# tonyjohnvan/ACE-Step-1.5

Measured on AMD Instinct MI355X. Metric: seconds/song (240 s audio, 27 DiT steps), lower is better.
Workload: dtype bf16

## Files before the change

ace-step-1.5_amd/csrc/gemm.hip:

```cpp
#include <hip/hip_ext.h>

#include "kernels.h"
#include "headpost.h"

namespace acehip {
namespace {

constexpr int BK = 64;
constexpr int GROUP_M = 8;

#ifdef GEMM_STAMPS
constexpr int STAMP_WG = 16384;
__device__ unsigned long long g_gemm_stamps[STAMP_WG * 2 * 8];
__device__ __forceinline__ void stamp(int slot, int i, unsigned long long v) {
    if (slot < STAMP_WG * 2) {
        asm volatile("" : "+v"(v));
        g_gemm_stamps[slot * 8 + i] = v;
    }
}
#define GSTAMP_AT(slot, i)                                                                       \
    do {                                                                                         \
        if ((threadIdx.x & 255) == 0 && threadIdx.x < 512) stamp((slot) * 2 + (threadIdx.x >> 8), i, __builtin_amdgcn_s_memtime()); \
    } while (0)
#define GSTAMP_REAL_AT(slot, i)                                                                  \
// ... 465 lines not shown
        asm volatile("s_getreg_b32 %0, hwreg(HW_REG_XCC_ID)" : "=s"(xcc));
        if ((threadIdx.x & 255) == 0) {
            stamp(slot * 2 + (threadIdx.x >> 8), 6, ((unsigned long long)wg << 32) | xcc);
            stamp(slot * 2 + (threadIdx.x >> 8), 7, blockIdx.x);
        }
    }
#endif
}

template <int BM>
struct PPSrcPtr {
    static constexpr int NA = BM / 64, NB = 4;
    const bf16_t *pa[NA], *pb[NB];
    __device__ __forceinline__ void set(const GemmArgs &a, int m0, int n0, int wave, int lane) {
#pragma unroll
        for (int i = 0; i < NA; ++i) {
            const int r = (wave + 8 * i) * 8 + (lane >> 3);
            const int c = (lane & 7) ^ ((r >> 1) & 7);
            pa[i] = a.A + (int64_t)min(m0 + r, a.M - 1) * a.lda + c * 8;
        }
#pragma unroll
        for (int i = 0; i < NB; ++i) {
            const int r = (wave + 8 * i) * 8 + (lane >> 3);
            const int c = (lane & 7) ^ (((BM + r) >> 1) & 7);
            pb[i] = a.W + (int64_t)(n0 + r) * a.ldw + c * 8;
        }
    }
    __device__ __forceinline__ void dmaA(int i, int k0, char *dst) const { glds16(pa[i] + k0, dst); }
    __device__ __forceinline__ void dmaB(int i, int k0, char *dst) const { glds16(pb[i] + k0, dst); }
};

__device__ __forceinline__ void glds16_s(const char *sbase, uint32_t voff, char *lds_dst) {
    const uint32_t la = (uint32_t)(uintptr_t)(const __attribute__((address_space(3))) char *)lds_dst;
    asm volatile("s_mov_b32 m0, %0\n\ts_nop 0\n\tglobal_load_lds_dwordx4 %1, %2" ::"s"(la), "v"(voff), "s"(sbase)
                 : "memory");
}

template <int BM>
struct PPSrcOff {
    static constexpr int NA = BM / 64, NB = 4;
    const char *ba, *bb;
    uint32_t oa[NA], ob, bstep;
    __device__ __forceinline__ void set(const GemmArgs &a, int m0, int n0, int wave, int lane) {
        ba = (const char *)(a.A + (int64_t)m0 * a.lda);
        bb = (const char *)(a.W + (int64_t)n0 * a.ldw);
        bstep = 64u * (uint32_t)a.ldw * 2u;
        const int r0 = wave * 8 + (lane >> 3);
        const uint32_t c16 = (uint32_t)((lane & 7) ^ ((r0 >> 1) & 7)) * 16u;
        ob = (uint32_t)r0 * (uint32_t)a.ldw * 2u + c16;
        const int last = a.M - 1 - m0;
#pragma unroll
        for (int i = 0; i < NA; ++i) oa[i] = (uint32_t)min(r0 + 64 * i, last) * (uint32_t)a.lda * 2u + c16;
    }
    __device__ __forceinline__ void dmaA(int i, int k0, char *dst) const { glds16_s(ba + (int64_t)k0 * 2, oa[i], dst); }
    __device__ __forceinline__ void dmaB(int i, int k0, char *dst) const {
        glds16_s(bb + (uint64_t)i * bstep + (int64_t)k0 * 2, ob, dst);
    }
};

template <int BM, int EPI, typename Src>
__device__ __forceinline__ void pp_stageA(const GemmArgs &a, char *lds, const Src &src, int wave, int buf, int k0) {
    constexpr int BUF = (BM + 256) * 128;
    char *b = lds + buf * BUF;
    int ko = k0;
    if constexpr (EPI == EPI_CONV) {
        const int cin = a.conv_cin, tap = k0 / cin;
        ko = k0 + tap * (a.conv_dil - 1) * cin + a.conv_a0 * cin;
    }
#pragma unroll
    for (int i = 0; i < Src::NA; ++i) src.dmaA(i, ko, b + (wave + 8 * i) * 1024);
}
template <int BM, typename Src>
__device__ __forceinline__ void pp_stageB(char *lds, const Src &src, int wave, int buf, int k0) {
    constexpr int BUF = (BM + 256) * 128;
    char *b = lds + buf * BUF + BM * 128;
#pragma unroll
    for (int i = 0; i < Src::NB; ++i) src.dmaB(i, k0, b + (wave + 8 * i) * 1024);
}
__device__ __forceinline__ void pp_bar() {
    __builtin_amdgcn_sched_barrier(0);
    __builtin_amdgcn_s_barrier();
    __builtin_amdgcn_sched_barrier(0);
}
template <int BM, int EPI, typename Src>
__device__ __forceinline__ void pp_prologue_issue(const GemmArgs &a, char *lds, const Src &src, int wave) {
    pp_stageB<BM>(lds, src, wave, 0, 0);
    pp_stageA<BM, EPI>(a, lds, src, wave, 0, 0);
    if (a.K > BK) pp_stageB<BM>(lds, src, wave, 1, BK);
}

constexpr int PP_SWIGLU_STORES = 256 / 2 / 16;

template <int BM, int EPI, bool PERSIST, typename Src>
__device__ __forceinline__ void pp_main(const GemmArgs &a, char *lds, const Src &src, f32x4 (&acc)[BM / 32][4],
                                        int slot, int pend) {
    constexpr int BN = 256, TM = BM / 2, SM = TM / 16, SMH = SM / 2;
    constexpr int ROWS = BM + BN, BUF = ROWS * 128;
    constexpr int NB = BN / 64;
    static_assert(SM % 2 == 0, "A half must be whole 16-row sub-tiles");
    const int tid = threadIdx.x, lane = tid & 63;
    int wave = tid >> 6;
    if constexpr (PERSIST) wave = __builtin_amdgcn_readfirstlane(wave);
    const int wr = wave >> 2, wc = wave & 3;
    auto stageA = [&](int buf, int k0) { pp_stageA<BM, EPI>(a, lds, src, wave, buf, k0); };
    auto stageB = [&](int buf, int k0) { pp_stageB<BM>(lds, src, wave, buf, k0); };
    auto bar = [] { pp_bar(); };

#pragma unroll
    for (int i = 0; i < SM; ++i)
#pragma unroll
        for (int j = 0; j < 4; ++j) acc[i][j] = f32x4{0.f, 0.f, 0.f, 0.f};

    const int fr = lane & 15, fc = lane >> 4;
    const int arow = wr * TM, brow = BM + wc * 64;

    const int nk = a.K / BK;
    if constexpr (!PERSIST) {
        stageB(0, 0);
        stageA(0, 0);
        if (nk > 1) {
            stageB(1, BK);
            asm volatile("s_waitcnt vmcnt(%0)" ::"n"(NB) : "memory");
        } else {
            asm volatile("s_waitcnt vmcnt(0)" ::: "memory");
        }
    } else {
        if (pend < 0) pp_prologue_issue<BM, EPI>(a, lds, src, wave);
        __builtin_amdgcn_sched_barrier(0);
        if (pend > 0) {
            if (nk > 1) asm volatile("s_waitcnt vmcnt(%0)" ::"n"(NB + PP_SWIGLU_STORES) : "memory");
            else asm volatile("s_waitcnt vmcnt(%0)" ::"n"(PP_SWIGLU_STORES) : "memory");
        } else {
            if (nk > 1) asm volatile("s_waitcnt vmcnt(%0)" ::"n"(NB) : "memory");
            else asm volatile("s_waitcnt vmcnt(0)" ::: "memory");
        }
    }
    bar();
    if (wr == 1) bar();
    GSTAMP_AT(slot, 1);

    {
    bf16x8 xa[SMH][2], bf[4][2];
    auto readA = [&](const char *b, int h) {
#pragma unroll
        for (int i = 0; i < SMH; ++i)
#pragma unroll
            for (int ks = 0; ks < 2; ++ks)
                xa[i][ks] = *(const bf16x8 *)(b + swz(arow + (h * SMH + i) * 16 + fr, ks * 4 + fc));
    };
    auto mma = [&](int h) {
        __builtin_amdgcn_sched_barrier(0);
        __builtin_amdgcn_s_setprio(1);
#pragma unroll
        for (int ks = 0; ks < 2; ++ks)
#pragma unroll
            for (int i = 0; i < SMH; ++i)
#pragma unroll
                for (int j = 0; j < 4; ++j)
                    acc[h * SMH + i][j] = __builtin_amdgcn_mfma_f32_16x16x32_bf16(bf[j][ks], xa[i][ks], acc[h * SMH + i][j], 0, 0, 0);
        __builtin_amdgcn_s_setprio(0);
    };
    for (int kt = 0; kt < nk; ++kt) {
        const char *b = lds + (kt & 1) * BUF;
#pragma unroll
        for (int j = 0; j < 4; ++j)
#pragma unroll
            for (int ks = 0; ks < 2; ++ks) bf[j][ks] = *(const bf16x8 *)(b + swz(brow + j * 16 + fr, ks * 4 + fc));
        readA(b, 0);
        if (kt + 1 < nk) stageA((kt + 1) & 1, (kt + 1) * BK);
        asm volatile("s_waitcnt lgkmcnt(0)" ::: "memory");
        bar();
        mma(0);
        bar();
        readA(b, 1);
        if (kt + 2 < nk) {
            stageB(kt & 1, (kt + 2) * BK);
            asm volatile("s_waitcnt vmcnt(%0) lgkmcnt(0)" ::"n"(NB) : "memory");
        } else {
            asm volatile("s_waitcnt vmcnt(0) lgkmcnt(0)" ::: "memory");
        }
        bar();
        mma(1);
        bar();
    }
    }
    if (wr == 0) bar();
    GSTAMP_AT(slot, 2);
}

template <int BM, int EPI>
__device__ __forceinline__ void pp_epilogue(const GemmArgs &a, char *lds, const f32x4 (&acc)[BM / 32][4], int m0, int n0) {
    constexpr int TM = BM / 2, SM = TM / 16, BUF = (BM + 256) * 128;
    const int tid = threadIdx.x, lane = tid & 63, wave = tid >> 6;
    const int wr = wave >> 2, wc = wave & 3;
    const int fr = lane & 15, fc = lane >> 4;
    const int arow = wr * TM;
    if constexpr (EPI == EPI_HEADPOST && BM == 256) {
#pragma unroll
        for (int hf = 0; hf < 2; ++hf)
            headpost_epilogue<128, 8, 2 * BUF, 2>(a, lds, m0 + hf * 128, n0, wave, lane, [&](bf16_t *st, int pitch) {
                if (wr != hf) return;
#pragma unroll
                for (int i = 0; i < SM; ++i)
#pragma unroll
                    for (int j = 0; j < 4; ++j) {
                        float o[4] = {acc[i][j][0], acc[i][j][1], acc[i][j][2], acc[i][j][3]};
                        *(uint2 *)(st + (i * 16 + fr) * pitch + wc * 64 + j * 16 + fc * 4) = pack4(o);
                    }
            });
        return;
    } else if constexpr (EPI == EPI_HEADPOST) {
        headpost_epilogue<BM, 8, 2 * BUF, 2>(a, lds, m0, n0, wave, lane, [&](bf16_t *st, int pitch) {
#pragma unroll
            for (int i = 0; i < SM; ++i)
#pragma unroll
                for (int j = 0; j < 4; ++j) {
                    float o[4] = {acc[i][j][0], acc[i][j][1], acc[i][j][2], acc[i][j][3]};
                    *(uint2 *)(st + (arow + i * 16 + fr) * pitch + wc * 64 + j * 16 + fc * 4) = pack4(o);
                }
        });
        return;
    }

    epilogue_tile<SM, 4, EPI>(a, acc, m0 + arow, n0 + wc * 64, fr, fc);
}

template <int BM, int EPI>
__device__ __forceinline__ void gemm_pp_body(const GemmArgs &a, char *lds, int bid) {
    GSTAMP(0);
    GSTAMP_REAL(4);
    const int tid = threadIdx.x, lane = tid & 63, wave = tid >> 6;
    int m0, n0;
    pp_tile_origin<BM>(a, bid, blockIdx.x, m0, n0);
    PPSrcPtr<BM> src;
    src.set(a, m0, n0, wave, lane);
    f32x4 acc[BM / 32][4];
    pp_main<BM, EPI, false>(a, lds, src, acc, blockIdx.x, -1);
    pp_epilogue<BM, EPI>(a, lds, acc, m0, n0);
    if constexpr (EPI == EPI_HEADPOST) return;
#ifdef GEMM_STAMPS
    asm volatile("s_waitcnt vmcnt(0)" ::: "memory");
#endif
    GSTAMP(3);
    GSTAMP_REAL(5);
}

template <int EPI>
__global__ __launch_bounds__(512, 1) void gemm_pp_persist_kernel(GemmArgs a, GemmArgs t, int nmain, int ntot) {
    static_assert(EPI == EPI_SWIGLU, "the early prologue needs an epilogue that leaves LDS alone and a known store count");
    __shared__ __attribute__((aligned(16))) char lds[pp_lds_bytes<256>()];
    const int tid = threadIdx.x, lane = tid & 63, wave = __builtin_amdgcn_readfirstlane(tid >> 6);
    const int G = gridDim.x;
    int i = blockIdx.x;
    int pend = -1;
    int m0 = 0, n0 = 0;
    GSTAMP_AT(i, 0);
    GSTAMP_REAL_AT(i, 4);
    PPSrcOff<256> src;
    PPSrcOff<128> tsrc;
    if (i < nmain) {
        pp_tile_origin<256>(a, i, i, m0, n0);
        src.set(a, m0, n0, wave, lane);
    }
    for (; i < nmain; i += G) {
        f32x4 acc[8][4];
        pp_main<256, EPI, true>(a, lds, src, acc, i, pend);
        const int cm0 = m0, cn0 = n0, nx = i + G;
        pend = cm0 + 256 <= a.M ? 1 : 0;
        if (nx < ntot) {
            GSTAMP_AT(nx, 0);
            GSTAMP_REAL_AT(nx, 4);
        }
        if (nx < nmain) {
            pp_tile_origin<256>(a, nx, nx, m0, n0);
            src.set(a, m0, n0, wave, lane);
            pp_prologue_issue<256, EPI>(a, lds, src, wave);
        } else if (nx < ntot) {
            pp_tile_origin<128>(t, nx - nmain, nx, m0, n0);
            tsrc.set(t, m0, n0, wave, lane);
            pp_prologue_issue<128, EPI>(t, lds, tsrc, wave);
        }
        __builtin_amdgcn_sched_barrier(0);
        pp_epilogue<256, EPI>(a, lds, acc, cm0, cn0);
        __builtin_amdgcn_sched_barrier(0);
        GSTAMP_AT(i, 3);
        GSTAMP_REAL_AT(i, 5);
    }
    for (; i < ntot; i += G) {
        if (pend < 0) {
            pp_tile_origin<128>(t, i - nmain, i, m0, n0);
            tsrc.set(t, m0, n0, wave, lane);
        }
        f32x4 acc[4][4];
        pp_main<128, EPI, true>(t, lds, tsrc, acc, i, pend);
        pend = -1;
        pp_epilogue<128, EPI>(t, lds, acc, m0, n0);
#ifdef GEMM_STAMPS
        asm volatile("s_waitcnt vmcnt(0)" ::: "memory");
#endif
        GSTAMP_AT(i, 3);
        GSTAMP_REAL_AT(i, 5);
        if (i + G < ntot) {
            GSTAMP_AT(i + G, 0);
            GSTAMP_REAL_AT(i + G, 4);
        }
    }
}

template <int BM, int EPI>
__global__ __launch_bounds__(512, 1) void gemm_pp_kernel(GemmArgs a) {
    __shared__ __attribute__((aligned(16))) char lds[pp_lds_bytes<BM>()];
    gemm_pp_body<BM, EPI>(a, lds, blockIdx.x);
}

template <int EPI>
__global__ __launch_bounds__(512, 1) void gemm_pp_split_kernel(GemmArgs a, GemmArgs t, int nmain) {
    __shared__ __attribute__((aligned(16))) char lds[pp_lds_bytes<256>()];
    if ((int)blockIdx.x < nmain) gemm_pp_body<256, EPI>(a, lds, blockIdx.x);
    else gemm_pp_body<128, EPI>(t, lds, blockIdx.x - nmain);
}

template <int BM, int BN, int EPI, int NH = 0>
__global__ __launch_bounds__(256 + 64 * NH, 1) void gemm_w4_kernel(GemmArgs a) {
    constexpr int TM = BM / 2, TN = BN / 2, SM = TM / 16, SN = TN / 16;
    constexpr int ROWS = BM + BN, STAGE = ROWS * 128;
    constexpr int NS = 3 * STAGE <= 160 * 1024 ? 3 : 2;
    constexpr int PW = ROWS / 32;
    static_assert(ROWS % 32 == 0, "staging must split evenly over 4 waves");
    __shared__ __attribute__((aligned(16))) char lds[NS * STAGE];

    GSTAMP(0);
    GSTAMP_REAL(4);
    const int tid = threadIdx.x, lane = tid & 63, wave = tid >> 6;
    const int wm = wave >> 1, wn = wave & 1;
    const int tilesM = (a.M + BM - 1) / BM, tilesN = a.N / BN;
    const int nwg = tilesM * tilesN;
    const int wg = xcd_remap(blockIdx.x, nwg);
    const int per_group = GROUP_M * tilesN;
    const int gid = wg / per_group, first_m = gid * GROUP_M;
    const int gsz = min(tilesM - first_m, GROUP_M);
    const int tm = first_m + (wg % per_group) % gsz;
    const int tn = (wg % per_group) / gsz;
    const int m0 = tm * BM, n0 = tn * BN;
    const int nk = a.K / BK;

    if constexpr (NH > 0) {
        if (__builtin_amdgcn_readfirstlane(wave) >= 4) {
            constexpr int PPH = 4 * PW / NH;
            static_assert((4 * PW) % NH == 0 && (NS - 1) * PPH < 64, "helper pieces / vmcnt field");
            const int h = wave - 4;
            const bf16_t *hs[PPH];
#pragma unroll
            for (int i = 0; i < PPH; ++i) {
                const int q = h + NH * i, r = q * 8 + (lane >> 3);
                const int c = (lane & 7) ^ ((r >> 1) & 7);
                if (r < BM) hs[i] = a.A + (int64_t)min(m0 + r, a.M - 1) * a.lda + c * 8;
                else hs[i] = a.W + (int64_t)(n0 + r - BM) * a.ldw + c * 8;
            }
            auto fill = [&](int buf, int k0) {
#pragma unroll
                for (int i = 0; i < PPH; ++i) glds16(hs[i] + k0, lds + buf * STAGE + (h + NH * i) * 1024);
            };
            for (int t = 0; t < NS; ++t) fill(t, min(t, nk - 1) * BK);
            asm volatile("s_waitcnt vmcnt(%0)" ::"n"((NS - 1) * PPH) : "memory");
            __builtin_amdgcn_s_barrier();
            for (int kt = 0; kt < nk; ++kt) {
                asm volatile("s_waitcnt vmcnt(%0)" ::"n"((NS - 2) * PPH) : "memory");
                __builtin_amdgcn_s_barrier();
                asm volatile("" ::: "memory");
                fill(kt % NS, min(kt + NS, nk - 1) * BK);
            }
            asm volatile("s_waitcnt vmcnt(0)" ::: "memory");
            if constexpr (EPI == EPI_HEADPOST) {
                __syncthreads();
                __syncthreads();
            }
            return;
        }
    }
// ... 134 lines not shown
            if constexpr (BM == 256 || BM == 192 || BM == 128) {
                gemm_pp_kernel<BM, EPI_HEADPOST><<<tiles, 512, 0, s>>>(a);
                break;
            }
            return fail(-1, "gemm: head-post epilogue needs the 256-, 192- or 128-row ping-pong tile");
        default: return fail(-1, "gemm: bad epilogue");
    }
    HIP_TRY(hipGetLastError());
    return 0;
}

template <int BM, int BN, int WM, int WN, int STAGES, int NH = 0>
int launch(const GemmArgs &a, hipStream_t s) {
    if (a.N % BN) return fail(-1, "gemm: N not a multiple of the tile");
    const int tiles = ((a.M + BM - 1) / BM) * (a.N / BN);
    constexpr int NT = WM * WN * 64 + 64 * NH;
    switch (a.epi) {
        case EPI_STORE: gemm_kernel<BM, BN, WM, WN, STAGES, EPI_STORE, NH><<<tiles, NT, 0, s>>>(a); break;
        case EPI_GATED_RES: gemm_kernel<BM, BN, WM, WN, STAGES, EPI_GATED_RES, NH><<<tiles, NT, 0, s>>>(a); break;
        case EPI_RES: gemm_kernel<BM, BN, WM, WN, STAGES, EPI_RES, NH><<<tiles, NT, 0, s>>>(a); break;
        case EPI_SWIGLU: klaunch(gemm_kernel<BM, BN, WM, WN, STAGES, EPI_SWIGLU, NH>, dim3(tiles), dim3(NT), s, a); break;
        default: return fail(-1, "gemm: bad epilogue for this variant");
    }
    HIP_TRY(hipGetLastError());
    return 0;
}

}

int gemm_variant(const GemmArgs &a, int variant, hipStream_t s) {
    switch (variant) {
        case 0: return launch<128, 128, 2, 2, 2>(a, s);
        case 7: return launch_pp<256>(a, s);
        case 8: return launch_pp<192>(a, s);
        case 9: return launch_pp<128>(a, s);
        case 13: return knobs().gemm_helpers ? launch_w4<192, 128, 2>(a, s) : launch_w4<192, 128>(a, s);
        case 16: return launch<128, 64, 4, 1, 4>(a, s);
        case 17: return launch<128, 64, 4, 1, 4, 2>(a, s);
        default: return fail(-1, "gemm: bad variant (0, 7, 8, 9, 13, 16, 17)");
    }
}

#ifdef GEMM_STAMPS
}
extern "C" int acehip_diag_gemm_stamps(void *host, int n_wg) {
    n_wg = std::min(n_wg, acehip::STAMP_WG);
    HIP_TRY(hipMemcpyFromSymbol(host, HIP_SYMBOL(acehip::g_gemm_stamps), (size_t)n_wg * 2 * 8 * 8));
    return 0;
}
extern "C" int acehip_diag_gemm_stamps_clear(void) {
    void *p = nullptr;
    HIP_TRY(hipGetSymbolAddress(&p, HIP_SYMBOL(acehip::g_gemm_stamps)));
    HIP_TRY(hipMemset(p, 0, sizeof(acehip::g_gemm_stamps)));
    return 0;
}
namespace acehip {
#endif

bool gemm_ext_events(hipEvent_t start, hipEvent_t stop) {
    const bool consumed = g_ext_ev.stop && !g_ext_ev.start;
    g_ext_ev.start = start;
    g_ext_ev.stop = stop;
    return consumed;
}

static int num_cus() {
    static int n = 0;
    if (!n) {
        int dev = 0;
        if (hipGetDevice(&dev) != hipSuccess ||
            hipDeviceGetAttribute(&n, hipDeviceAttributeMultiprocessorCount, dev) != hipSuccess || n <= 0)
            n = 256;
    }
    return n;
}
static int plan_cus() {
    const int cap = knobs().gemm_cus, n = num_cus();
    return cap > 0 && cap < n ? cap : n;
}

static int launch_pp_persist(const GemmArgs &hd, const GemmArgs &tl, int nmain, int ntail, hipStream_t s) {
    const int grid = std::min(plan_cus(), nmain + ntail);
    if (ntail > grid) return fail(-1, "gemm: persistent walk with more tail tiles than workgroups");
    klaunch(gemm_pp_persist_kernel<EPI_SWIGLU>, dim3(grid), dim3(512), s, hd, tl, nmain, nmain + ntail);
    HIP_TRY(hipGetLastError());
    return 0;
}

static bool use_w4s(int64_t M, int N) {
    if (N % 128) return false;
    const int cus = num_cus();
    const int64_t t = ((M + 191) / 192) * (N / 128);
    return t <= cus && t * 4 >= (int64_t)cus * 3;
}

int gemm_pick_variant(int64_t M, int N) {
    if (use_w4s(M, N) && (N % 256 || ((M + 191) / 192) * (N / 256) <= num_cus() / 2)) return 13;
    if (N % 256) return 0;
    const int cus = plan_cus();
    const int64_t t7 = ((M + 255) / 256) * (N / 256), t8 = ((M + 191) / 192) * (N / 256);
    if (t8 <= cus / 2) return 0;
    const int64_t t9 = ((M + 127) / 128) * (N / 256);
    if (t8 <= cus && t9 <= cus) return 9;
    const double c7 = (double)((t7 + cus - 1) / cus) * 1.093, c8 = (double)((t8 + cus - 1) / cus);
    return c7 < c8 ? 7 : 8;
}

static int splitk_finish(const GemmArgs &a, const GemmArgs &p, int splits, hipStream_t s);

static int splitk_bn(const GemmArgs &) {
    const int f = knobs().splitk_bn;
    if (f) return f == 64 ? 64 : 128;
    return 64;
}
static void fill_defer(const GemmArgs &a, int splits, RowAdd *defer);
static int gemm_splitk(const GemmArgs &a, int splits, hipStream_t s, RowAdd *defer = nullptr) {
    GemmArgs p = a;
    const int nk = a.K / BK;
    p.kper = (nk + splits - 1) / splits;
    splits = (nk + p.kper - 1) / p.kper;
    const int bn = splitk_bn(a);
    const int tiles = ((a.M + 127) / 128) * (a.N / bn);
    if (bn == 64) gemm_kernel<128, 64, 4, 1, 3, EPI_PARTIAL><<<dim3(tiles, splits), 256, 0, s>>>(p);
    else if (a.N <= 4096) gemm_kernel<128, 128, 2, 2, 3, EPI_PARTIAL><<<dim3(tiles, splits), 256, 0, s>>>(p);
    else gemm_kernel<128, 128, 2, 2, 2, EPI_PARTIAL><<<dim3(tiles, splits), 256, 0, s>>>(p);
    HIP_TRY(hipGetLastError());
    if (defer) {
        fill_defer(a, splits, defer);
        return 0;
    }
    return splitk_finish(a, p, splits, s);
}

static void fill_defer(const GemmArgs &a, int splits, RowAdd *defer) {
    defer->xw = a.C;
    defer->part = (const float *)a.ws;
    defer->splits = splits;
    defer->prows = a.M;
    defer->plane = (int64_t)a.M * a.N;
    defer->gate = a.epi == EPI_GATED_RES ? a.gate : nullptr;
    defer->gate_bstride = a.gate_bstride;
    defer->gate_rpb = a.epi == EPI_GATED_RES ? a.rows_per_batch : 1;
}

static int splitk_finish(const GemmArgs &a, const GemmArgs &p, int splits, hipStream_t s) {
    if (a.epi == EPI_HEADPOST && knobs().splitk_fuse) {
        HeadPostArgs h = a.hp;
        h.part = (const float *)a.ws;
        h.splits = splits;
        h.plane = (int64_t)a.M * a.N;
        h.ld_src = a.N;
        return head_post(h, s);
    }
    bf16_t *out = a.C;
    int64_t ldo = a.ldc;
    if (a.epi == EPI_HEADPOST) {
        out = (bf16_t *)((char *)a.ws + (size_t)splits * a.M * a.N * 4);
        ldo = a.N;
    }
    const int nout = a.epi == EPI_SWIGLU ? a.N / 2 : a.N;
    const int64_t thr = (int64_t)a.M * nout / 4;
    splitk_epilogue_kernel<<<(unsigned)((thr + 255) / 256), 256, 0, s>>>(p, splits, out, ldo);
    HIP_TRY(hipGetLastError());
    if (a.epi == EPI_HEADPOST) {
        HeadPostArgs h = a.hp;
        h.src = out;
        h.ld_src = a.N;
        return head_post(h, s);
    }
    return 0;
}

static int gemm_tail_split(const GemmArgs &a, int v, hipStream_t s) {
    if (a.epi != EPI_SWIGLU && a.epi != EPI_STORE && a.epi != EPI_HEADPOST) return 1;
    if (!knobs().gemm_tailsplit) return 1;
    const int BMv = v == 7 ? 256 : 192, cus = plan_cus();
    const int64_t nN = a.N / 256, tiles = (int64_t)((a.M + BMv - 1) / BMv) * nN;
    const int64_t full = tiles / cus, rem = tiles - full * cus;
    if (full < 1 || rem == 0 || rem * 5 > (int64_t)cus * 3) return 1;
    const int64_t M1 = (full * cus / nN) * BMv;
    if (M1 <= 0 || M1 >= a.M) return 1;
    if (((a.M - M1 + 127) / 128) * (a.N / 128) > 2 * (int64_t)cus) return 1;
    GemmArgs hd = a;
    hd.M = (int)M1;
    GemmArgs tl = a;
    tl.M = a.M - (int)M1;
    tl.A = a.A + M1 * a.lda;
    if (a.epi == EPI_HEADPOST) tl.hp.m_off += (int)M1;
    else tl.C = a.C + M1 * a.ldc;
    const bool pp128 = a.N % 256 == 0 && ((tl.M + 127) / 128) * nN <= cus;
    if (a.epi == EPI_HEADPOST && !pp128) return 1;
    if (pp128 && v == 7) {
        const int nmain = (int)(full * cus / nN * nN), ntail = ((tl.M + 127) / 128) * (int)nN;
        if (a.epi == EPI_SWIGLU && knobs().gemm_persist && nmain == (hd.M / 256) * (int)nN && hd.M % 256 == 0)
            return launch_pp_persist(hd, tl, nmain, ntail, s);
        if (nmain % 8 == 0 && nmain == (hd.M / 256) * (int)nN && hd.M % 256 == 0) {
            if (a.epi == EPI_SWIGLU) klaunch(gemm_pp_split_kernel<EPI_SWIGLU>, dim3(nmain + ntail), dim3(512), s, hd, tl, nmain);
            else if (a.epi == EPI_HEADPOST) gemm_pp_split_kernel<EPI_HEADPOST><<<nmain + ntail, 512, 0, s>>>(hd, tl, nmain);
            else gemm_pp_split_kernel<EPI_STORE><<<nmain + ntail, 512, 0, s>>>(hd, tl, nmain);
            HIP_TRY(hipGetLastError());
            return 0;
        }
    }
    int rc = gemm_variant(hd, v, s);
    if (rc) return rc;
    return gemm_variant(tl, pp128 ? 9 : 0, s);
}

static int launch_conv64(const GemmArgs &a, hipStream_t s) {
    const int tiles = ((a.M + 63) / 64) * (a.N / 256);
    gemm_pp_kernel<64, EPI_CONV><<<tiles, 512, 0, s>>>(a);
    HIP_TRY(hipGetLastError());
    return 0;
}

int gemm_conv(const GemmArgs &a, hipStream_t s) {
    if (a.epi != EPI_CONV || (!a.C && !a.Cs) || (a.Cs && (!a.sa || !a.sib)) || a.conv_cin <= 0 || a.conv_dil < 1 ||
        a.conv_ostride < 1 || a.conv_cout <= 0 || a.conv_cout % 8 || a.N % a.conv_cout || a.conv_lout <= 0 || a.M <= 0)
        return fail(-1, "gemm_conv: EPI_CONV with an output, snake parameters and conv geometry required");
    if (a.N % 256 || a.conv_cin % BK || a.K % a.conv_cin || a.lda != a.conv_cin || a.ldw != a.K || a.ldc != a.conv_cout)
        return fail(-1, "gemm_conv: N % 256, cin % 64, K = taps·cin and dense layouts required");
    if (a.res && (a.N != a.conv_cout || a.ldr != a.N || a.conv_ostride != 1 || a.conv_ooff != 0 || a.conv_lout != a.M))
        return fail(-1, "gemm_conv: a residual needs one phase with output row = m");
    if ((int64_t)((a.M + 255) / 256) * (a.N / 256) >= (1ll << 31)) return fail(-1, "gemm_conv: grid too large");
    const int64_t t256 = (int64_t)((a.M + 255) / 256) * (a.N / 256);
    if (t256 * 4 <= num_cus()) return launch_conv64(a, s);
    if (t256 * 2 <= num_cus()) return launch_pp<128>(a, s);
    return launch_pp<256>(a, s);
}

int gemm(const GemmArgs &a, hipStream_t s, RowAdd *defer) {
    if (defer) defer->part = nullptr;
    if (a.M <= 0) return 0;
    if (a.N % 128 || a.K % BK || a.K <= 0)
        return fail(-1, "gemm: N%128 / K%64 violated (M=" + std::to_string(a.M) + " N=" +
                            std::to_string(a.N) + " K=" + std::to_string(a.K) + ")");
    if ((a.lda | a.ldw | a.ldc) % 8) return fail(-1, "gemm: leading dims must be multiples of 8");
    if (a.epi == EPI_GATED_RES && (!a.gate || a.rows_per_batch <= 0)) return fail(-1, "gemm: gate");
    if ((a.epi == EPI_GATED_RES || a.epi == EPI_RES) && !a.res) return fail(-1, "gemm: res");
    if (a.epi == EPI_HEADPOST) {
        const HeadPostArgs &h = a.hp;
        if (a.N % 256 || h.S <= 0 || (int64_t)h.B * h.S != a.M || (h.nq + h.nk + h.nv) * 128 != a.N ||
            h.S_dst < h.S || (h.S_dst_q && h.S_dst_q < h.S) || (h.nq && !h.qw) || (h.nk && !h.kw) || (h.cos == nullptr) != (h.sin == nullptr))
            return fail(-1, "gemm: head-post arguments inconsistent with the GEMM shape");
    }
    const Knobs &kn = knobs();
    const bool dfr = defer && kn.splitk_fuse && (a.epi == EPI_GATED_RES || a.epi == EPI_RES) && a.res == a.C &&
                     a.ldr == a.ldc && a.ldc == a.N;
    if (a.epi == EPI_SWIGLU && a.M <= 128 && a.N % 64 == 0 && kn.smallm_wholek) return gemm_variant(a, kn.smallm_wholek == 2 ? 17 : 16, s);
    if (a.ws && a.N % 128 == 0 && a.K % BK == 0 && (a.N % 256 == 0 || a.epi != EPI_HEADPOST)) {
        const int cus = num_cus();
        const int64_t tiles = ((a.M + 127) / 128) * (a.N / 128);
        const int nk = a.K / BK;
        if (tiles * 2 <= cus && nk >= 8) {
            const int64_t tb = ((a.M + 127) / 128) * (a.N / splitk_bn(a));
            int splits = (int)std::min<int64_t>(std::min<int64_t>(16, nk / 4), (cus + tb - 1) / tb);
            const size_t need = (size_t)splits * a.M * a.N * 4 + (size_t)a.M * a.N * 2;
            if (splits >= 2 && need <= a.ws_bytes) return gemm_splitk(a, splits, s, dfr ? defer : nullptr);
        }
    }
    if (a.epi == EPI_HEADPOST) {
        const int64_t t192 = (int64_t)((a.M + 191) / 192) * (a.N / 256);
        const bool small = t192 * 2 <= num_cus();
        if (small && use_w4s(a.M, a.N)) return gemm_variant(a, 13, s);
        if (small && a.ws && (size_t)a.M * a.N * 2 <= a.ws_bytes) {
            GemmArgs st = a;
            st.epi = EPI_STORE;
            st.bias = nullptr;
            st.C = (bf16_t *)a.ws;
            st.ldc = a.N;
            int rc = gemm_variant(st, 0, s);
            if (rc) return rc;
            HeadPostArgs hh = a.hp;
            hh.src = st.C;
            hh.ld_src = a.N;
            return head_post(hh, s);
        }
        if (kn.gemm_hp_tail && a.N % 256 == 0) {
            const int cus = num_cus();
            const int64_t nN = a.N / 256, t7 = ((a.M + 255) / 256) * nN, t8 = ((a.M + 191) / 192) * nN;
            const double c_split = (double)(t7 / cus) * 1.093 + 0.6, c8 = (double)((t8 + cus - 1) / cus);
            if (t7 >= cus && c_split < c8) {
                const int rc = gemm_tail_split(a, 7, s);
                if (rc <= 0) return rc;
            }
        }
        return gemm_variant(a, 8, s);
    }
    const int v = gemm_pick_variant(a.M, a.N);
    if (v == 7 || v == 8) {
        const int rc = gemm_tail_split(a, v, s);
        if (rc <= 0) return rc;
    }
    if (v == 7 && a.epi == EPI_SWIGLU && knobs().gemm_persist) {
        const int64_t tiles = (int64_t)((a.M + 255) / 256) * (a.N / 256);
        if (tiles > plan_cus() && tiles < (1ll << 30)) return launch_pp_persist(a, a, (int)tiles, 0, s);
    }
    return gemm_variant(a, v, s);
}

}
```

ace-step-1.5_amd/csrc/kernels.h:

```cpp
#pragma once
#include "common.h"

namespace acehip {

struct Knobs {
    int gemm_tailsplit = 1;
    int gemm_helpers = 1;
    int splitk_fuse = 1;
    int splitk_bn = 0;
    int smallm_wholek = 2;
    int attn_pw = 2;
    int attn_persist = 1;
    int attn_small = 1;
    int attn_small_mask = 1;
    int attn_small_causal = 1;
    int attn_cus = 0;
    int attn_streamk = 1;
    int fuse_rowadd = 1;
    int dit_dedup = 1;
    int dit_graph = 0;
    int gemm_persist = 1;
    int gemm_cus = 0;
    int gemm_hp_tail = 1;
    int convt = 1;
    int conv7 = 2;
    int convp = 3;
    int ru7 = 2;
    int vae_snake_in = 1;
    int kv_group_kib = 262144;
    unsigned gen = 0;
};
const Knobs &knobs();

struct HeadPostArgs {
    const bf16_t *src; int64_t ld_src;
    int B, S;
    int nq, nk, nv;
    const bf16_t *qw, *kw;
    const bf16_t *cos, *sin;
    bf16_t *q, *k, *v;
    int S_dst;
    float eps;
    const float *part = nullptr; int splits = 0; int64_t plane = 0;
    int m_off = 0;
    int S_dst_q = 0;
};
enum GemmEpi {
    EPI_STORE = 0,
    EPI_GATED_RES = 1,
    EPI_RES = 2,
    EPI_SWIGLU = 3,
    EPI_HEADPOST = 4,
};


struct GemmArgs {
    const bf16_t *A; int64_t lda;
    const bf16_t *W; int64_t ldw;
    bf16_t *C; int64_t ldc;
    int M, N, K;
    int epi;
    const bf16_t *bias;
    const bf16_t *res; int64_t ldr;
    const bf16_t *gate; int64_t gate_bstride; int rows_per_batch;
    HeadPostArgs hp;
    void *ws; size_t ws_bytes;
    int kper;
    const float *sa, *sib;
    bf16_t *Cs;
    int conv_cin, conv_dil, conv_a0, conv_ostride, conv_ooff, conv_cout;
    int64_t conv_lout;
};
constexpr int EPI_PARTIAL = 5;
constexpr int EPI_CONV = 6;
constexpr size_t GEMM_WS_BYTES = (size_t)48 << 20;
struct RowAdd;
int gemm(const GemmArgs &a, hipStream_t s, RowAdd *defer = nullptr);
int gemm_variant(const GemmArgs &a, int variant, hipStream_t s);
int gemm_conv(const GemmArgs &a, hipStream_t s);
bool gemm_ext_events(hipEvent_t start, hipEvent_t stop);

int gemv_small(const bf16_t *x, int64_t ldx, const bf16_t *W, const bf16_t *bias, bf16_t *y,
               int64_t ldy, int M, int N, int K, int act, hipStream_t s, bf16_t *act_scratch = nullptr);
int bcast_rows(const bf16_t *src, int64_t n, bf16_t *dst, int rows, hipStream_t s);
int timestep_sinusoid(const float *t, const float *t_r, int t_stride, int use_diff, int Bc,
                      const float *freqs, bf16_t *emb, hipStream_t s);
int add_bf16(const bf16_t *a, const bf16_t *b, bf16_t *out, int64_t n, hipStream_t s);
int modulation(const bf16_t *tables, int n_tables, int rows, const bf16_t *proj, int Bc, int D,
               bf16_t *mod, hipStream_t s);
int pack_patches(const bf16_t *xt, const bf16_t *ctx, int Bx, int Bc, int T, int S, bf16_t *X,
                 hipStream_t s);
int gather_head_row(const bf16_t *V, int KV, int Le, int H, bf16_t *out, hipStream_t s);
int add_row_bcast(bf16_t *X, const bf16_t *c, int rows, int D, hipStream_t s);
int copy_cols(const bf16_t *src, int64_t lds, bf16_t *dst, int64_t ldd, int M, int C, hipStream_t s);
int crop_rows(const bf16_t *src, int Bc, int rows_src, int rows_dst, int C, bf16_t *dst,
              hipStream_t s);

struct RowAdd {
    bf16_t *xw = nullptr;
    const bf16_t *v = nullptr;
    int from = 0;
    const float *part = nullptr;
    int splits = 0, prows = 0;
    int64_t plane = 0;
// ... 91 lines not shown
```

ace-step-1.5_amd/csrc/knobs.hip:

```cpp
#include <atomic>
#include <cstdlib>
#include <mutex>

#include "kernels.h"
#include "../../include/acehip.h"

namespace acehip {
namespace {

int env_int(const char *name, int dflt) {
    const char *e = getenv(name);
    return (e && *e) ? atoi(e) : dflt;
}

Knobs read_env() {
    Knobs k;
    k.gemm_tailsplit = env_int("ACEHIP_GEMM_TAILSPLIT", 1);
    k.gemm_helpers = env_int("ACEHIP_GEMM_HELPERS", 1);
    k.splitk_fuse = env_int("ACEHIP_SPLITK_FUSE", 1);
    k.splitk_bn = env_int("ACEHIP_SPLITK_BN", 0);
    k.smallm_wholek = env_int("ACEHIP_SMALLM_WHOLEK", 2);
    k.attn_pw = env_int("ACEHIP_ATTN_PW", 2);
    k.attn_persist = env_int("ACEHIP_ATTN_PERSIST", 1);
    k.attn_small = env_int("ACEHIP_ATTN_SMALL", 1);
    k.attn_small_mask = env_int("ACEHIP_ATTN_SMALL_MASK", 1);
    k.attn_small_causal = env_int("ACEHIP_ATTN_SMALL_CAUSAL", 1);
    k.attn_cus = env_int("ACEHIP_ATTN_CUS", 0);
    k.attn_streamk = env_int("ACEHIP_ATTN_STREAMK", 1);
    k.fuse_rowadd = env_int("ACEHIP_FUSE_ROWADD", 1);
    k.dit_dedup = env_int("ACEHIP_DIT_DEDUP", 1);
    k.dit_graph = env_int("ACEHIP_DIT_GRAPH", 0);
    k.conv7 = env_int("ACEHIP_CONV7", 2);
    k.convt = env_int("ACEHIP_CONVT", 1);
    k.gemm_hp_tail = env_int("ACEHIP_GEMM_HPTAIL", 1);
    k.gemm_persist = env_int("ACEHIP_GEMM_PERSIST", 1);
    k.gemm_cus = env_int("ACEHIP_GEMM_CUS", 0);
    k.convp = env_int("ACEHIP_CONVP", 3);
    k.ru7 = env_int("ACEHIP_RU7", 2);
    k.kv_group_kib = env_int("ACEHIP_KV_GROUP_KIB", 262144);
    k.vae_snake_in = env_int("ACEHIP_VAE_SNAKE_IN", 1);
    if (k.kv_group_kib <= 0) k.kv_group_kib = 262144;
    return k;
}

std::mutex g_mu;
Knobs g_knobs;
std::atomic<bool> g_loaded{false};

}

const Knobs &knobs() {
    if (!g_loaded.load(std::memory_order_acquire)) {
        std::lock_guard<std::mutex> lk(g_mu);
        if (!g_loaded.load(std::memory_order_relaxed)) {
            g_knobs = read_env();
            g_loaded.store(true, std::memory_order_release);
        }
    }
    return g_knobs;
}

}

extern "C" int acehip_reload_knobs(void) {
    std::lock_guard<std::mutex> lk(acehip::g_mu);
    const unsigned gen = acehip::g_knobs.gen + 1;
    acehip::g_knobs = acehip::read_env();
    acehip::g_knobs.gen = gen;
    acehip::g_loaded.store(true, std::memory_order_release);
    return 0;
}
```

Baseline: 0.5337.

## Extend persistent pipelined GEMM walk to headpost and conv epilogues

Generalizes the persistent GEMM kernel, which issues the next tile's prologue loads while the current tile's epilogue stores drain, from SwiGLU-only to headpost and conv epilogues. Headpost gets a separate LDS staging region so its epilogue does not clobber the next tile's prefetched buffers, with the second B stage issued after a barrier. Conv gets its own outstanding-store accounting. Heuristics now use plan_cus instead of num_cus, and the gemm_persist knob becomes a bitmask defaulting to all three paths. The cost is more LDS for headpost, extra barriers, and tighter vmcnt bookkeeping that could stall or race if the store counts are wrong.

```diff
diff --git a/ace-step-1.5_amd/csrc/gemm.hip b/ace-step-1.5_amd/csrc/gemm.hip
--- a/ace-step-1.5_amd/csrc/gemm.hip
+++ b/ace-step-1.5_amd/csrc/gemm.hip
@@ -571,14 +571,16 @@
     __builtin_amdgcn_s_barrier();
     __builtin_amdgcn_sched_barrier(0);
 }
-template <int BM, int EPI, typename Src>
+template <int BM, int EPI, bool B1 = true, typename Src>
 __device__ __forceinline__ void pp_prologue_issue(const GemmArgs &a, char *lds, const Src &src, int wave) {
     pp_stageB<BM>(lds, src, wave, 0, 0);
     pp_stageA<BM, EPI>(a, lds, src, wave, 0, 0);
-    if (a.K > BK) pp_stageB<BM>(lds, src, wave, 1, BK);
+    if constexpr (B1)
+        if (a.K > BK) pp_stageB<BM>(lds, src, wave, 1, BK);
 }
 
 constexpr int PP_SWIGLU_STORES = 256 / 2 / 16;
+constexpr int PP_CONV_STORES = 256 / 2 / 16 * 2;
 
 template <int BM, int EPI, bool PERSIST, typename Src>
 __device__ __forceinline__ void pp_main(const GemmArgs &a, char *lds, const Src &src, f32x4 (&acc)[BM / 32][4],
@@ -587,9 +589,10 @@
     constexpr int ROWS = BM + BN, BUF = ROWS * 128;
     constexpr int NB = BN / 64;
     static_assert(SM % 2 == 0, "A half must be whole 16-row sub-tiles");
-    const int tid = threadIdx.x, lane = tid & 63;
-    int wave = tid >> 6;
+    const int tid = threadIdx.x;
+    int lane = tid & 63, wave = tid >> 6;
     if constexpr (PERSIST) wave = __builtin_amdgcn_readfirstlane(wave);
+    if constexpr (PERSIST && EPI != EPI_SWIGLU) asm volatile("" : "+v"(lane));
     const int wr = wave >> 2, wc = wave & 3;
     auto stageA = [&](int buf, int k0) { pp_stageA<BM, EPI>(a, lds, src, wave, buf, k0); };
     auto stageB = [&](int buf, int k0) { pp_stageB<BM>(lds, src, wave, buf, k0); };
@@ -616,7 +619,14 @@
     } else {
         if (pend < 0) pp_prologue_issue<BM, EPI>(a, lds, src, wave);
         __builtin_amdgcn_sched_barrier(0);
-        if (pend > 0) {
+        if (EPI == EPI_HEADPOST && pend == 0) {
+        } else if (EPI == EPI_CONV && pend == 2 * PP_CONV_STORES) {
+            if (nk > 1) asm volatile("s_waitcnt vmcnt(%0)" ::"n"(NB + 2 * PP_CONV_STORES) : "memory");
+            else asm volatile("s_waitcnt vmcnt(%0)" ::"n"(2 * PP_CONV_STORES) : "memory");
+        } else if (EPI == EPI_CONV && pend > 0) {
+            if (nk > 1) asm volatile("s_waitcnt vmcnt(%0)" ::"n"(NB + PP_CONV_STORES) : "memory");
+            else asm volatile("s_waitcnt vmcnt(%0)" ::"n"(PP_CONV_STORES) : "memory");
+        } else if (pend > 0) {
             if (nk > 1) asm volatile("s_waitcnt vmcnt(%0)" ::"n"(NB + PP_SWIGLU_STORES) : "memory");
             else asm volatile("s_waitcnt vmcnt(%0)" ::"n"(PP_SWIGLU_STORES) : "memory");
         } else {
@@ -677,10 +687,12 @@
     GSTAMP_AT(slot, 2);
 }
 
-template <int BM, int EPI>
+template <int BM, int EPI, bool DRAIN = false>
 __device__ __forceinline__ void pp_epilogue(const GemmArgs &a, char *lds, const f32x4 (&acc)[BM / 32][4], int m0, int n0) {
     constexpr int TM = BM / 2, SM = TM / 16, BUF = (BM + 256) * 128;
-    const int tid = threadIdx.x, lane = tid & 63, wave = tid >> 6;
+    int tid = threadIdx.x;
+    if constexpr (DRAIN) asm volatile("" : "+v"(tid));
+    const int lane = tid & 63, wave = tid >> 6;
     const int wr = wave >> 2, wc = wave & 3;
     const int fr = lane & 15, fc = lane >> 4;
     const int arow = wr * TM;
@@ -688,6 +700,8 @@
 #pragma unroll
         for (int hf = 0; hf < 2; ++hf)
             headpost_epilogue<128, 8, 2 * BUF, 2>(a, lds, m0 + hf * 128, n0, wave, lane, [&](bf16_t *st, int pitch) {
+                if constexpr (DRAIN)
+                    if (hf == 0) asm volatile("s_waitcnt vmcnt(0)" ::: "memory");
                 if (wr != hf) return;
 #pragma unroll
                 for (int i = 0; i < SM; ++i)
@@ -734,10 +748,35 @@
     GSTAMP_REAL(5);
 }
 
+constexpr int PP_HP_STAGE_OFF = (256 + 256) * 128;
+constexpr int PP_HP_STAGE = 128 * (2 * 128 + 8) * 2;
+template <int EPI>
+constexpr int pp_persist_lds_bytes() {
+    return EPI == EPI_HEADPOST ? PP_HP_STAGE_OFF + PP_HP_STAGE : pp_lds_bytes<256>();
+}
+static_assert(PP_HP_STAGE == 67584, "the staging half-tile of headpost_epilogue<128, 8, ·, 2>");
+static_assert(PP_HP_STAGE_OFF >= (256 + 256) * 128 && PP_HP_STAGE_OFF >= (128 + 256) * 128,
+              "the staging tile lies above buffer 0 of a main and of a tail tile");
+static_assert(pp_persist_lds_bytes<EPI_HEADPOST>() <= 160 * 1024, "LDS of one CU");
+
+template <int EPI>
+__device__ __forceinline__ int pp_pend_stores(const GemmArgs &a, int m0) {
+    if (EPI == EPI_HEADPOST || m0 + 256 > a.M) return 0;
+    if constexpr (EPI == EPI_CONV) {
+        const int64_t lo = (int64_t)m0 * a.conv_ostride + a.conv_ooff;
+        const int64_t hi = (int64_t)(m0 + 255) * a.conv_ostride + a.conv_ooff + (a.N / a.conv_cout - 1);
+        if (lo < 0 || hi >= a.conv_lout) return 0;
+        return ((a.C ? 1 : 0) + (a.Cs ? 1 : 0)) * PP_CONV_STORES;
+    }
+    return 1;
+}
+
 template <int EPI>
 __global__ __launch_bounds__(512, 1) void gemm_pp_persist_kernel(GemmArgs a, GemmArgs t, int nmain, int ntot) {
-    static_assert(EPI == EPI_SWIGLU, "the early prologue needs an epilogue that leaves LDS alone and a known store count");
-    __shared__ __attribute__((aligned(16))) char lds[pp_lds_bytes<256>()];
+    static_assert(EPI == EPI_SWIGLU || EPI == EPI_CONV || EPI == EPI_HEADPOST,
+                  "the early prologue needs an epilogue whose LDS use and store count are accounted for");
+    constexpr bool HP = EPI == EPI_HEADPOST;
+    __shared__ __attribute__((aligned(16))) char lds[pp_persist_lds_bytes<EPI>()];
     const int tid = threadIdx.x, lane = tid & 63, wave = __builtin_amdgcn_readfirstlane(tid >> 6);
     const int G = gridDim.x;
     int i = blockIdx.x;
@@ -755,7 +794,7 @@
         f32x4 acc[8][4];
         pp_main<256, EPI, true>(a, lds, src, acc, i, pend);
         const int cm0 = m0, cn0 = n0, nx = i + G;
-        pend = cm0 + 256 <= a.M ? 1 : 0;
+        pend = pp_pend_stores<EPI>(a, cm0);
         if (nx < ntot) {
             GSTAMP_AT(nx, 0);
             GSTAMP_REAL_AT(nx, 4);
@@ -763,18 +802,35 @@
         if (nx < nmain) {
             pp_tile_origin<256>(a, nx, nx, m0, n0);
             src.set(a, m0, n0, wave, lane);
-            pp_prologue_issue<256, EPI>(a, lds, src, wave);
+            pp_prologue_issue<256, EPI, !HP>(a, lds, src, wave);
         } else if (nx < ntot) {
-            pp_tile_origin<128>(t, nx - nmain, nx, m0, n0);
-            tsrc.set(t, m0, n0, wave, lane);
-            pp_prologue_issue<128, EPI>(t, lds, tsrc, wave);
+            if constexpr (EPI != EPI_CONV) {
+                pp_tile_origin<128>(t, nx - nmain, nx, m0, n0);
+                tsrc.set(t, m0, n0, wave, lane);
+                pp_prologue_issue<128, EPI, !HP>(t, lds, tsrc, wave);
+            }
         }
         __builtin_amdgcn_sched_barrier(0);
-        pp_epilogue<256, EPI>(a, lds, acc, cm0, cn0);
+        pp_epilogue<256, EPI, HP>(a, HP ? lds + PP_HP_STAGE_OFF : lds, acc, cm0, cn0);
         __builtin_amdgcn_sched_barrier(0);
+        if constexpr (HP) {
+            asm volatile("s_waitcnt lgkmcnt(0)" ::: "memory");
+            pp_bar();
+            m0 = __builtin_amdgcn_readfirstlane(m0);
+            n0 = __builtin_amdgcn_readfirstlane(n0);
+            if (nx < nmain) {
+                src.set(a, m0, n0, wave, lane);
+                if (a.K > BK) pp_stageB<256>(lds, src, wave, 1, BK);
+            } else if (nx < ntot) {
+                tsrc.set(t, m0, n0, wave, lane);
+                if (t.K > BK) pp_stageB<128>(lds, tsrc, wave, 1, BK);
+            }
+            __builtin_amdgcn_sched_barrier(0);
+        }
         GSTAMP_AT(i, 3);
         GSTAMP_REAL_AT(i, 5);
     }
+    if constexpr (EPI != EPI_CONV)
     for (; i < ntot; i += G) {
         if (pend < 0) {
             pp_tile_origin<128>(t, i - nmain, i, m0, n0);
@@ -784,6 +840,10 @@
         pp_main<128, EPI, true>(t, lds, tsrc, acc, i, pend);
         pend = -1;
         pp_epilogue<128, EPI>(t, lds, acc, m0, n0);
+        if constexpr (HP) {
+            asm volatile("s_waitcnt lgkmcnt(0)" ::: "memory");
+            pp_bar();
+        }
 #ifdef GEMM_STAMPS
         asm volatile("s_waitcnt vmcnt(0)" ::: "memory");
 #endif
@@ -1084,7 +1144,10 @@
 static int launch_pp_persist(const GemmArgs &hd, const GemmArgs &tl, int nmain, int ntail, hipStream_t s) {
     const int grid = std::min(plan_cus(), nmain + ntail);
     if (ntail > grid) return fail(-1, "gemm: persistent walk with more tail tiles than workgroups");
-    klaunch(gemm_pp_persist_kernel<EPI_SWIGLU>, dim3(grid), dim3(512), s, hd, tl, nmain, nmain + ntail);
+    if (hd.epi == EPI_SWIGLU) klaunch(gemm_pp_persist_kernel<EPI_SWIGLU>, dim3(grid), dim3(512), s, hd, tl, nmain, nmain + ntail);
+    else if (hd.epi == EPI_HEADPOST) gemm_pp_persist_kernel<EPI_HEADPOST><<<grid, 512, 0, s>>>(hd, tl, nmain, nmain + ntail);
+    else if (hd.epi == EPI_CONV && ntail == 0) gemm_pp_persist_kernel<EPI_CONV><<<grid, 512, 0, s>>>(hd, tl, nmain, nmain);
+    else return fail(-1, "gemm: no persistent walk for this epilogue");
     HIP_TRY(hipGetLastError());
     return 0;
 }
@@ -1194,7 +1257,8 @@
     if (a.epi == EPI_HEADPOST && !pp128) return 1;
     if (pp128 && v == 7) {
         const int nmain = (int)(full * cus / nN * nN), ntail = ((tl.M + 127) / 128) * (int)nN;
-        if (a.epi == EPI_SWIGLU && knobs().gemm_persist && nmain == (hd.M / 256) * (int)nN && hd.M % 256 == 0)
+        const int pbit = a.epi == EPI_SWIGLU ? 1 : a.epi == EPI_HEADPOST ? 2 : 0;
+        if ((knobs().gemm_persist & pbit) && nmain == (hd.M / 256) * (int)nN && hd.M % 256 == 0)
             return launch_pp_persist(hd, tl, nmain, ntail, s);
         if (nmain % 8 == 0 && nmain == (hd.M / 256) * (int)nN && hd.M % 256 == 0) {
             if (a.epi == EPI_SWIGLU) klaunch(gemm_pp_split_kernel<EPI_SWIGLU>, dim3(nmain + ntail), dim3(512), s, hd, tl, nmain);
@@ -1226,8 +1290,9 @@
         return fail(-1, "gemm_conv: a residual needs one phase with output row = m");
     if ((int64_t)((a.M + 255) / 256) * (a.N / 256) >= (1ll << 31)) return fail(-1, "gemm_conv: grid too large");
     const int64_t t256 = (int64_t)((a.M + 255) / 256) * (a.N / 256);
-    if (t256 * 4 <= num_cus()) return launch_conv64(a, s);
-    if (t256 * 2 <= num_cus()) return launch_pp<128>(a, s);
+    if (t256 * 4 <= plan_cus()) return launch_conv64(a, s);
+    if (t256 * 2 <= plan_cus()) return launch_pp<128>(a, s);
+    if ((knobs().gemm_persist & 4) && t256 > plan_cus() && t256 < (1ll << 30)) return launch_pp_persist(a, a, (int)t256, 0, s);
     return launch_pp<256>(a, s);
 }
 
@@ -1251,7 +1316,7 @@
                      a.ldr == a.ldc && a.ldc == a.N;
     if (a.epi == EPI_SWIGLU && a.M <= 128 && a.N % 64 == 0 && kn.smallm_wholek) return gemm_variant(a, kn.smallm_wholek == 2 ? 17 : 16, s);
     if (a.ws && a.N % 128 == 0 && a.K % BK == 0 && (a.N % 256 == 0 || a.epi != EPI_HEADPOST)) {
-        const int cus = num_cus();
+        const int cus = plan_cus();
         const int64_t tiles = ((a.M + 127) / 128) * (a.N / 128);
         const int nk = a.K / BK;
         if (tiles * 2 <= cus && nk >= 8) {
@@ -1263,7 +1328,7 @@
     }
     if (a.epi == EPI_HEADPOST) {
         const int64_t t192 = (int64_t)((a.M + 191) / 192) * (a.N / 256);
-        const bool small = t192 * 2 <= num_cus();
+        const bool small = t192 * 2 <= plan_cus();
         if (small && use_w4s(a.M, a.N)) return gemm_variant(a, 13, s);
         if (small && a.ws && (size_t)a.M * a.N * 2 <= a.ws_bytes) {
             GemmArgs st = a;
@@ -1279,13 +1344,15 @@
             return head_post(hh, s);
         }
         if (kn.gemm_hp_tail && a.N % 256 == 0) {
-            const int cus = num_cus();
+            const int cus = plan_cus();
             const int64_t nN = a.N / 256, t7 = ((a.M + 255) / 256) * nN, t8 = ((a.M + 191) / 192) * nN;
             const double c_split = (double)(t7 / cus) * 1.093 + 0.6, c8 = (double)((t8 + cus - 1) / cus);
             if (t7 >= cus && c_split < c8) {
                 const int rc = gemm_tail_split(a, 7, s);
                 if (rc <= 0) return rc;
             }
+            if ((kn.gemm_persist & 2) && t7 > cus && t7 % cus == 0 && (double)(t7 / cus) * 1.093 < c8 && t7 < (1ll << 30))
+                return launch_pp_persist(a, a, (int)t7, 0, s);
         }
         return gemm_variant(a, 8, s);
     }
@@ -1294,7 +1361,7 @@
         const int rc = gemm_tail_split(a, v, s);
         if (rc <= 0) return rc;
     }
-    if (v == 7 && a.epi == EPI_SWIGLU && knobs().gemm_persist) {
+    if (v == 7 && a.epi == EPI_SWIGLU && (knobs().gemm_persist & 1)) {
         const int64_t tiles = (int64_t)((a.M + 255) / 256) * (a.N / 256);
         if (tiles > plan_cus() && tiles < (1ll << 30)) return launch_pp_persist(a, a, (int)tiles, 0, s);
     }
diff --git a/ace-step-1.5_amd/csrc/kernels.h b/ace-step-1.5_amd/csrc/kernels.h
--- a/ace-step-1.5_amd/csrc/kernels.h
+++ b/ace-step-1.5_amd/csrc/kernels.h
@@ -19,7 +19,7 @@
     int fuse_rowadd = 1;
     int dit_dedup = 1;
     int dit_graph = 0;
-    int gemm_persist = 1;
+    int gemm_persist = 7;
     int gemm_cus = 0;
     int gemm_hp_tail = 1;
     int convt = 1;
diff --git a/ace-step-1.5_amd/csrc/knobs.hip b/ace-step-1.5_amd/csrc/knobs.hip
--- a/ace-step-1.5_amd/csrc/knobs.hip
+++ b/ace-step-1.5_amd/csrc/knobs.hip
@@ -33,7 +33,7 @@
     k.conv7 = env_int("ACEHIP_CONV7", 2);
     k.convt = env_int("ACEHIP_CONVT", 1);
     k.gemm_hp_tail = env_int("ACEHIP_GEMM_HPTAIL", 1);
-    k.gemm_persist = env_int("ACEHIP_GEMM_PERSIST", 1);
+    k.gemm_persist = env_int("ACEHIP_GEMM_PERSIST", 7);
     k.gemm_cus = env_int("ACEHIP_GEMM_CUS", 0);
     k.convp = env_int("ACEHIP_CONVP", 3);
     k.ru7 = env_int("ACEHIP_RU7", 2);
```

Result: no change. 0.5325, median of 6 (-0.2%).
